# y2w-oc/CMR-Agent

Hardware: AMD Instinct MI355X
Metric: registration iters/sec (KITTI 352x1216 img + 16384 pts, 1 geo forward + 10 agent steps) (higher is better)
Workload: dtype f32; 1 GPU; BASELINE.json configs[1]: KittiConfig, batch 8 per GPU, 16384 pts, 352x1216 image, 10 agent steps, fp32, hash-filled weights; batch_per_gpu=8, parallelism=batch sharding, no data-path collective

## Files before the change

cmr_agent_amd/csrc/agent.hip:

```cpp
#include "cmr_common.h"

namespace {

__global__ __launch_bounds__(256) void project_scatter_kernel(const float* __restrict__ pc4, const float* __restrict__ feat,
                                                              const uint8_t* __restrict__ overlap,
                                                              const float* __restrict__ pose ,
                                                              const float* __restrict__ Kmat ,
                                                              const float* __restrict__ mean4 ,
                                                              float* __restrict__ acc, float* __restrict__ cnt,
                                                              float* __restrict__ state3d, int B, int N, int h, int w) {
  const int lane = threadIdx.x & 63;
  const int64_t p0 = ((int64_t)blockIdx.x * 4 + (threadIdx.x >> 6)) * 4;
  const int64_t total = (int64_t)B * N;
  for (int q = 0; q < 4; ++q) {
    const int64_t p = p0 + q;
    if (p >= total) return;
    const int b = (int)(p / N);
    const f32x4 pt = *reinterpret_cast<const f32x4*>(pc4 + p * 4);
    const float* R = pose + b * 16;
    const float* Kb = Kmat + b * 9;
    const float mx = mean4[b * 4 + 0], my = mean4[b * 4 + 1], mz = mean4[b * 4 + 2];
    const float cx = pt[0] - mx, cy = pt[1] - my, cz = pt[2] - mz;
    const float tx = (R[0] * cx + R[1] * cy + R[2] * cz) + mx + R[3];
    const float ty = (R[4] * cx + R[5] * cy + R[6] * cz) + my + R[7];
// ... 46 lines not shown
__device__ __forceinline__ void obs_mark_reach(uint8_t* __restrict__ map, int r, int b, int yi, int xi, int h, int w) {
  const int tiles_y = (h + 7) >> 3, tiles_x = (w + 15) >> 4;
  const int ya = (yi - r > 0 ? yi - r : 0) >> 3, yb = (yi + r) >> 3 < tiles_y ? (yi + r) >> 3 : tiles_y - 1;
  const int xa = (xi - r > 0 ? xi - r : 0) >> 4, xb = (xi + r) >> 4 < tiles_x ? (xi + r) >> 4 : tiles_x - 1;
  uint8_t* m = map + (int64_t)b * tiles_y * tiles_x;
  m[ya * tiles_x + xa] = 1;
  m[ya * tiles_x + xb] = 1;
  m[yb * tiles_x + xa] = 1;
  m[yb * tiles_x + xb] = 1;
}

__global__ __launch_bounds__(256) void obs_project_kernel(const float* __restrict__ pc4, const uint8_t* __restrict__ overlap,
                                                          const float* __restrict__ pose, const float* __restrict__ Kmat,
                                                          const float* __restrict__ mean4, float* __restrict__ proj, float* __restrict__ cnt,
                                                          int32_t* __restrict__ cell, float* __restrict__ state3d, int B, int N, int h, int w,
                                                          uint8_t* __restrict__ reach1, uint8_t* __restrict__ reach2) {
  const int64_t p = (int64_t)blockIdx.x * 256 + threadIdx.x;
  if (p >= (int64_t)B * N) return;
  const int32_t prev = cell[p];
  if (prev >= 0) {
    f32x4* row = reinterpret_cast<f32x4*>(proj + (int64_t)prev * 64);
    const f32x4 z = {0.f, 0.f, 0.f, 0.f};
#pragma unroll
    for (int i = 0; i < 16; ++i) row[i] = z;
    cnt[prev] = 0.f;
  }
  const int b = (int)(p / N);
  const f32x4 pt = *reinterpret_cast<const f32x4*>(pc4 + p * 4);
  const float* R = pose + b * 16;
  const float* Kb = Kmat + b * 9;
  const float mx = mean4[b * 4 + 0], my = mean4[b * 4 + 1], mz = mean4[b * 4 + 2];
// ... 6 lines not shown
  const float zc = Kb[6] * tx + Kb[7] * ty + Kb[8] * tz;
  u = u / zc;
  v = v / zc;
  const bool inside = (u >= 0.f) && (u <= (float)(w - 1)) && (v >= 0.f) && (v <= (float)(h - 1)) && (zc > 0.f);
  const bool ov = overlap[p] != 0;
  *reinterpret_cast<f32x4*>(state3d + p * 8) = f32x4{pt[0], pt[1], pt[2], ov ? 1.f : 0.f};
  *reinterpret_cast<f32x4*>(state3d + p * 8 + 4) = f32x4{inside ? 1.f : 0.f, 0.f, 0.f, 0.f};
  int32_t c = -1;
  if (ov && inside) {
    const int xi = (int)rintf(u), yi = (int)rintf(v);
    c = (int32_t)((int64_t)b * h * w + (int64_t)yi * w + xi);
    if (reach1) {
      obs_mark_reach(reach1, 1, b, yi, xi, h, w);
      obs_mark_reach(reach2, 2, b, yi, xi, h, w);
    }
  }
  cell[p] = c;
}

__global__ __launch_bounds__(256) void obs_count_kernel(const int32_t* __restrict__ cell, float* __restrict__ cnt, int64_t total) {
  const int64_t p = (int64_t)blockIdx.x * 256 + threadIdx.x;
  if (p >= total) return;
  const int32_t c = cell[p];
  if (c >= 0) atomicAdd(cnt + c, 1.f);
}

__global__ __launch_bounds__(256) void obs_scatter_kernel(const float* __restrict__ feat, const int32_t* __restrict__ cell,
                                                          const float* __restrict__ cnt, float* __restrict__ proj, int64_t total) {
  const int lane = threadIdx.x & 63;
  const int64_t p0 = ((int64_t)blockIdx.x * 4 + (threadIdx.x >> 6)) * 4;
// ... 107 lines not shown
extern "C" int cmr_project_scatter_f32(const float* pc4, const float* feat, const uint8_t* overlap, const float* pose,
                                       const float* Kmat, const float* mean4, float* acc, float* cnt, float* state3d,
                                       int B, int N, int h, int w, int zero_first, hipStream_t stream) {
  CMR_REQUIRE(pc4 && feat && overlap && pose && Kmat && mean4 && acc && cnt && state3d && B > 0 && N > 0 && h > 0 && w > 0);
  const int64_t cells = (int64_t)B * h * w;
  if (zero_first) {
    if (hipMemsetAsync(acc, 0, cells * 64 * sizeof(float), stream) != hipSuccess) return CMR_ELAUNCH;
    if (hipMemsetAsync(cnt, 0, cells * sizeof(float), stream) != hipSuccess) return CMR_ELAUNCH;
  }
  const int64_t total = (int64_t)B * N;
  hipLaunchKernelGGL(project_scatter_kernel, dim3((unsigned)((total + 15) / 16)), dim3(256), 0, stream, pc4, feat, overlap,
                     pose, Kmat, mean4, acc, cnt, state3d, B, N, h, w);
  return cmr_launch_status();
}

extern "C" int cmr_observation_proj_reach_f32(const float* pc4, const float* feat, const uint8_t* overlap, const float* pose, const float* Kmat,
                                              const float* mean4, float* proj, float* cnt, int32_t* cell, float* state3d, int B, int N, int h,
                                              int w, uint8_t* reach1, uint8_t* reach2, hipStream_t stream) {
  CMR_REQUIRE(pc4 && feat && overlap && pose && Kmat && mean4 && proj && cnt && cell && state3d && B > 0 && N > 0 && h > 0 && w > 0);
  CMR_REQUIRE((int64_t)B * h * w < 0x7fffffff && cmr_aligned16(proj) && cmr_aligned16(state3d) && cmr_aligned16(pc4));
  CMR_REQUIRE((reach1 == nullptr) == (reach2 == nullptr));
  const int64_t total = (int64_t)B * N;
  const unsigned per_point = (unsigned)((total + 255) / 256);
  hipLaunchKernelGGL(obs_project_kernel, dim3(per_point), dim3(256), 0, stream, pc4, overlap, pose, Kmat, mean4, proj, cnt, cell, state3d, B, N,
                     h, w, reach1, reach2);
  hipLaunchKernelGGL(obs_count_kernel, dim3(per_point), dim3(256), 0, stream, (const int32_t*)cell, cnt, total);
  hipLaunchKernelGGL(obs_scatter_kernel, dim3((unsigned)((total + 15) / 16)), dim3(256), 0, stream, feat, (const int32_t*)cell,
                     (const float*)cnt, proj, total);
  return cmr_launch_status();
}

extern "C" int cmr_observation_proj_f32(const float* pc4, const float* feat, const uint8_t* overlap, const float* pose, const float* Kmat,
                                        const float* mean4, float* proj, float* cnt, int32_t* cell, float* state3d, int B, int N, int h,
                                        int w, hipStream_t stream) {
  return cmr_observation_proj_reach_f32(pc4, feat, overlap, pose, Kmat, mean4, proj, cnt, cell, state3d, B, N, h, w, nullptr, nullptr, stream);
}

extern "C" int cmr_observation_finalize_f32(const float* img_feat, float* acc, float* cnt, float* state2d,
                                            float* proj, int B, int h, int w, int write_img, int clear, hipStream_t stream) {
  CMR_REQUIRE(img_feat && acc && cnt && (state2d || proj) && B > 0 && h > 0 && w > 0);
  const int64_t cells = (int64_t)B * h * w;
  hipLaunchKernelGGL(observation_finalize_kernel, dim3((unsigned)((cells * 16 + 255) / 256)), dim3(256), 0, stream,
                     img_feat, acc, cnt, state2d, proj, cells, write_img, clear);
  return cmr_launch_status();
// ... 38 lines not shown
```

cmr_agent_amd/csrc/conv_wino.hip:

```cpp
#include "cmr_common.h"


namespace {

struct WinoArgs {
  const float* x; int B, H, W, Cin;
  const float* u;
  const float* bias; const float* res; const float* post;
  float* y; int Cout; float slope; int pool;
  float* stats;
  const float* bn_x; const float* bn_stat; float bn_slope;
};

constexpr int WT_TH = 8, WT_TW = 16;
constexpr int WT_HR = 10, WT_HC = 18;
constexpr int WT_KC = 32;
constexpr int WT_C4 = WT_KC / 4;
constexpr int WT_HALO_F4 = WT_HR * WT_HC * WT_C4;
constexpr int WT_HL = (WT_HALO_F4 + 255) / 256;
constexpr int WT_PITCH = 20;
constexpr int WT_SLOTS = WT_HR * WT_PITCH;
constexpr int WT_HALO_FLOATS = WT_SLOTS * WT_KC;
constexpr int WT_DMA = WT_SLOTS / 8;
constexpr int WT_DMA_PER_WAVE = (WT_DMA + 3) / 4;
// ... 279 lines not shown
}

constexpr int WS_T_OFF = 2 * WT_HALO_FLOATS;
constexpr int WS_T_ROW = 68;
constexpr int WS_SMEM_FLOATS = WS_T_OFF + 8 * 32 * WS_T_ROW;

__device__ __forceinline__ void ws_barrier_lds() { asm volatile("s_waitcnt lgkmcnt(0)\n\ts_barrier" ::: "memory"); }

#ifndef CMR_WS_STATS
#define CMR_WS_STATS 1
#endif
#ifndef CMR_WS_BNBWD
#define CMR_WS_BNBWD 0
#endif
constexpr bool WS_STATS = CMR_WS_STATS != 0, WS_BNBWD = CMR_WS_STATS != 0 && CMR_WS_BNBWD != 0;
struct WsList { const int* order; const int* nlive; const float* y0; };
template <int dbg, bool LIST>
__global__ __launch_bounds__(512, 1) void conv3x3_wino_ws_kernel(const WinoArgs a, const int tiles_x, const int tiles_y, const int ntiles, const WsList l) {
  extern __shared__ __attribute__((aligned(16))) float smem[];
  constexpr int NT = 2;
  constexpr int NMW = 4;
  const int tid = threadIdx.x, lane = tid & 63;
  const int wave = __builtin_amdgcn_readfirstlane(tid >> 6);
  const int nco = a.Cout / 64;
  const int nchunk = a.Cin / WT_KC;
  int nt = ntiles;
  if constexpr (LIST) {
    nt = __builtin_amdgcn_readfirstlane(*l.nlive);
    nt = nt < 0 ? 0 : (nt < ntiles ? nt : ntiles);
  }
  const int nk = (nt - (int)blockIdx.x + (int)gridDim.x - 1) / (int)gridDim.x;
// ... 397 lines not shown
        st_s[e] += cmr_xhalf(st_s[e]);
        st_q[e] += cmr_xor16(st_q[e]);
        st_q[e] += cmr_xhalf(st_q[e]);
      }
      if (lane < 16) {
        float* o = a.stats + ((int64_t)blockIdx.x * 4 + hw) * 128 + 4 * lane;
        *reinterpret_cast<f32x4*>(o) = st_s;
        *reinterpret_cast<f32x4*>(o + 64) = st_q;
      }
    }
  }
  if constexpr (LIST) {
    const int pw = a.pool == 2 ? WT_TW / 2 : WT_TW, pn = a.pool == 2 ? WT_TH * WT_TW / 4 : WT_TH * WT_TW;
    const int Hy = a.pool == 2 ? a.H >> 1 : a.H, Wy = a.pool == 2 ? a.W >> 1 : a.W;
    const int c4 = tid & 15;
    for (int s = nt + (int)blockIdx.x; s < ntiles; s += (int)gridDim.x) {
      int t = l.order[s];
      t = (unsigned)t < (unsigned)ntiles ? t : ntiles - 1;
      const int co0 = (t % nco) * 64; t /= nco;
      const int bx0 = (t % tiles_x) * pw; t /= tiles_x;
      const int by0 = (t % tiles_y) * (pn / pw);
      const int b = t / tiles_y;
      for (int p = tid >> 4; p < pn; p += 32) {
        const int py = by0 + p / pw, px = bx0 + p % pw;
        if (py >= Hy || px >= Wy) continue;
        const int64_t o = (((int64_t)b * Hy + py) * Wy + px) * a.Cout + co0 + 4 * c4;
        f32x4 v;
        if (l.y0) {
          v = *reinterpret_cast<const f32x4*>(l.y0 + o);
        } else {
          const f32x4 bsv = *reinterpret_cast<const f32x4*>(a.bias ? a.bias + co0 + 4 * c4 : wt_zero16);
// ... 134 lines not shown
    const int v = tid >= d ? cnt[tid - d] : 0;
    __syncthreads();
    cnt[tid] += v;
    __syncthreads();
  }
  const int total = cnt[1023];
  int live = cnt[tid] - n, dead = total + (lo - live);
  for (int i = lo; i < hi; ++i) {
    const int slot = reach[i] != 0 ? live++ : dead++;
    reach[i] = 0;
    for (int c = 0; c < nco; ++c) order[slot * nco + c] = i * nco + c;
  }
  if (tid == 0) *(blockIdx.x ? nlive2 : nlive1) = total * nco;
}

}

extern "C" int cmr_wino_tile_lists(uint8_t* reach1, uint8_t* reach2, int B, int H, int W, int Cout1, int Cout2, int* order1, int* nlive1,
                                   int* order2, int* nlive2, hipStream_t stream) {
  CMR_REQUIRE(reach1 && reach2 && order1 && nlive1 && order2 && nlive2 && B > 0 && H > 0 && W > 0);
  CMR_REQUIRE(Cout1 >= 64 && Cout1 % 64 == 0 && Cout2 >= 64 && Cout2 % 64 == 0);
  const int64_t ntile = (int64_t)((W + WT_TW - 1) / WT_TW) * ((H + WT_TH - 1) / WT_TH) * B;
  CMR_REQUIRE(ntile * (Cout1 / 64) < 0x3fffffff && ntile * (Cout2 / 64) < 0x3fffffff);
  hipLaunchKernelGGL(wino_tile_lists_kernel, dim3(2), dim3(1024), 0, stream, reach1, reach2, (int)ntile, Cout1 / 64, Cout2 / 64, order1, nlive1,
                     order2, nlive2);
  return cmr_launch_status();
}

extern "C" int cmr_conv3x3_wino_list_nhwc_f32(const float* x, int B, int H, int W, int Cin, const float* u, const float* bias, const float* res,
                                              float* y, int Cout, float slope, int pool, const int* order, const int* nlive, const float* y0,
                                              int cu_budget, int slices, hipStream_t stream) {
  CMR_REQUIRE(x && u && y && order && nlive && B > 0 && H > 0 && W > 0 && Cin % 32 == 0 && Cin >= 32 && Cout % 64 == 0 && Cout >= 64);
  CMR_REQUIRE(cmr_aligned16(x) && cmr_aligned16(u) && cmr_aligned16(y) && (!bias || cmr_aligned16(bias)) && (!res || cmr_aligned16(res)) &&
              (!y0 || cmr_aligned16(y0)));
  CMR_REQUIRE((pool == 1 || (pool == 2 && !res && y0)) && y0 != y);
  const int tiles_x = (W + WT_TW - 1) / WT_TW, tiles_y = (H + WT_TH - 1) / WT_TH;
  const int64_t ntiles64 = (int64_t)tiles_x * tiles_y * B * (Cout / 64);
  CMR_REQUIRE(2 * ntiles64 < 0x7fffffff);
  if (!(CMR_WINO_WS && Cin >= 64 && ntiles64 >= 200 && slope >= 0.f && slope <= 1.f)) return CMR_EUNSUPPORTED;
  const WinoArgs a{x, B, H, W, Cin, u, bias, res, nullptr, y, Cout, slope, pool};
  return launch_wino_ws_t<0, true>(a, tiles_x, tiles_y, ntiles64, cu_budget, slices, stream, WsList{order, nlive, y0});
}
```

cmr_agent_amd/environment/environment.py:

```python
import torch

from .. import ops
from ..models.CMRAgent import CMRAgent
from ..models.ImageResNet import to_nhwc
from ..models.PointNN import rows_from_bcl


DIRECT_PROJ = True


class _ObsContext:

    def __init__(self, data):
        cl = data.get('_cmr')
        pc = data['pc']
        self.B, _, self.N = pc.shape
        dev = pc.device
        if cl is not None and 'geo' in cl and cl['geo'].pc4.device == dev:
            self.pc4 = cl['geo'].pc4
        else:
            self.pc4 = ops.planar_to_rows(pc.contiguous(), 4)
        self.feat = cl['pc_geo_feat'] if cl is not None and 'pc_geo_feat' in cl else rows_from_bcl(data['pc_geo_feat'])
        ov = data['pc_overlap_pred']
        self.overlap = ov.contiguous().view(torch.uint8).view(-1) if ov.dtype == torch.bool else ov.to(torch.uint8).view(-1)
        self.overlap_src = ov
        self.img = cl['img_geo_feat'] if cl is not None and 'img_geo_feat' in cl else to_nhwc(data['img_geo_feat'])
        _, self.h, self.w, c = self.img.shape
        if c != 64:
            raise ValueError("observation kernels are instantiated for 64-d geometric features")
        self.K = data['K'].to(dev).contiguous()
        cen = data.get('_cmr_centroid')
        self.mean4 = cen[1] if (cen is not None and cen[0] is pc) else _centroid(pc, self.pc4)
        self.acc = self.cnt = None
        self.first = True
        self.proj = self.proj_cnt = self.proj_cell = None
        self.reach, self.obs_serial = None, 0
        self.agent_cache = {}
        self.dirty = False


def _context(data):
    ctx = data.get('_cmr_obs')
    if ctx is None or ctx.overlap_src is not data['pc_overlap_pred'] or ctx.pc4.device != data['pc'].device:
        ctx = _ObsContext(data)
        data['_cmr_obs'] = ctx
    return ctx


def _centroid(pcd, pc4=None):
    B, _, N = pcd.shape
# ... 30 lines not shown
    return poses


@torch.no_grad()
def observation_from_a_pose(data, RT, materialize_state_2d=True):
    ctx = _context(data)
    B, N, h, w = ctx.B, ctx.N, ctx.h, ctx.w
    dev = ctx.pc4.device
    state3d = torch.empty((B * N, 8), dtype=torch.float32, device=dev)
    if not materialize_state_2d and DIRECT_PROJ:
        if ctx.proj is None:
            ctx.proj = torch.zeros((B, h, w, 64), dtype=torch.float32, device=dev)
            ctx.proj_cnt = torch.zeros((B * h * w,), dtype=torch.float32, device=dev)
            ctx.proj_cell = torch.full((B * N,), -1, dtype=torch.int32, device=dev)
        sparse = CMRAgent.sparse_obs()
        if sparse and ctx.reach is None:
            ctx.reach = torch.zeros((2, B, (h + 7) // 8, (w + 15) // 16), dtype=torch.uint8, device=dev)
        ops.observation_proj(ctx.pc4, ctx.feat, ctx.overlap, RT.contiguous(), ctx.K, ctx.mean4, B, N, h, w, ctx.proj, ctx.proj_cnt,
                             ctx.proj_cell, state3d, reach=ctx.reach if sparse else None)
        ctx.obs_serial += 1
        ctx.agent_cache["reach"] = (ctx.reach, ctx.proj, ctx.obs_serial) if sparse else None
        obs2d = torch.empty((B, 128, h, w), dtype=torch.float32, device="meta")
        obs2d._cmr_split = (ctx.img, ctx.proj, ctx.agent_cache)
        return obs2d, state3d.view(B, N, 8)[:, :, :5].permute(0, 2, 1)
    state2d = torch.empty((B, h, w, 128), dtype=torch.float32, device=dev) if materialize_state_2d else None
    proj = torch.empty((B, h, w, 64), dtype=torch.float32, device=dev)
    if ctx.acc is None:
        ctx.acc = torch.zeros((B * h * w, 64), dtype=torch.float32, device=dev)
        ctx.cnt = torch.zeros((B * h * w,), dtype=torch.float32, device=dev)
    zero_first, ctx.dirty = ctx.dirty, True
    ops.project_scatter(ctx.pc4, ctx.feat, ctx.overlap, RT.contiguous(), ctx.K, ctx.mean4, B, N, h, w, ctx.acc, ctx.cnt,
                        state3d, zero_first=zero_first)
    ops.observation_finalize(ctx.img, ctx.acc, ctx.cnt, state2d, proj, B, h, w, True, clear=True)
    ctx.dirty = False
    obs2d = state2d.permute(0, 3, 1, 2) if state2d is not None else torch.empty((B, 128, h, w), dtype=torch.float32, device="meta")
    obs2d._cmr_split = (ctx.img, proj, ctx.agent_cache)
# ... 52 lines not shown
```

cmr_agent_amd/models/CMRAgent.py:

```python
import torch
import torch.nn as nn

from .. import ops
from ..utils.streams import fork_join
from . import _pack
from ._pack import Planned
from .ImageResNet import to_nhwc
from .PointNN import ConvBNReLURes1D

SLOPE = 0.01


def _mlp(sizes):
    layers = []
    for i in range(len(sizes) - 1):
        layers.append(nn.Linear(sizes[i], sizes[i + 1]))
        if i < len(sizes) - 2:
            layers.append(nn.LeakyReLU(inplace=True))
    return nn.Sequential(*layers)


class CMRAgent(Planned):
    def __init__(self, config):
        super().__init__()
# ... 66 lines not shown
                g = ops.colmax_partials(part, B, N // 32)
                b1b = ops.linear(g, ent["w1b"], ent["b1"])
                b2b = ops.linear(g, ent["wscb"], ent["b2"])
            last = i == 2
            r = ops.cbr_block(feat, ent["w1a"], b1b, ent["w2"], b2b, ent["wsca"], 0.2, rows_per_batch=N,
                              want_y=not last, want_colmax="partials")
            if r is None:
                return None
            feat, part = r
        return ops.colmax_partials(part, B, N // 32)

    FUSED_TAIL = True
    TAIL_T = True

    SPARSE_OBS = True

    @classmethod
    def sparse_obs(cls):
        return cls.SPARSE_OBS and ops.WINOGRAD and not ops.CONV_BF16

    def _tile_lists(self, cache, proj, c, u0, u1):
        mark = cache.get("reach")
        if mark is None or not self.sparse_obs() or self.training or mark[1] is not proj or u0 is None or u1 is None:
            return None
        B, h, w, cin = proj.shape
        if h % 2 or w % 2 or not (ops.wino_list_served(B, h, w, cin, c) and ops.wino_list_served(B, h, w, c, c)):
            return None
        if cache.get("lists_of") != mark[2]:
            cache["lists"] = (c, ops.wino_tile_lists(mark[0], B, h, w, c, c))
            cache["lists_of"] = mark[2]
        width, lists = cache["lists"]
        return lists if width == c else None

    def _embed_2d(self, state2d, B, split):
        p = self.plan()
        c = 2 * self.config.embed_dim
        x = state2d
        for stage, ((wa, ba, ua), (wb, bb, ub)) in enumerate(p["convs"]):
            if stage == 0 and split is not None:
                img_src, proj, cache = split
                tag = (id(self), id(p))
                if cache.get("tag") != tag:
                    wi, bi, ui = p["conv0_img"]
                    cache["val"] = ops.conv3x3(img_src, wi, bi, c, 1, 1.0, u=ui)
                    cache["tag"] = tag
                wp, _, up = p["conv0_proj"]
                lists = self._tile_lists(cache, proj, c, up, ub)
                if lists is not None:
                    if cache.get("tag0") != tag:
                        none = torch.zeros((1,), dtype=torch.int32, device=proj.device)
                        cache["x1_0"] = ops.conv3x3_wino_list(proj, up, None, c, SLOPE, lists[0][0], none, None, res=cache["val"])
                        cache["x2_0"] = ops.conv3x3(cache["x1_0"], wb, bb, c, 1, SLOPE, pool=2, u=ub)
                        cache["tag0"] = tag
                    (o1, n1), (o2, n2) = lists
                    x = ops.conv3x3_wino_list(proj, up, None, c, SLOPE, o1, n1, cache["x1_0"], res=cache["val"])
                    x = ops.conv3x3_wino_list(x, ub, bb, c, SLOPE, o2, n2, cache["x2_0"], pool=2)
                    continue
                x = ops.conv3x3(proj, wp, None, c, 1, SLOPE, res=cache["val"], u=up, out_bf16=True)
            else:
                x = ops.conv3x3(x, wa, ba, c, 1, SLOPE, u=ua, out_bf16=True)
            x = ops.conv3x3(x, wb, bb, c, 1, SLOPE, pool=2 if stage < 3 else 1, u=ub, out_bf16=stage < 3)
            if stage == 3:
                kh, kw = self.config.image_H // 8, self.config.image_W // 8
                if (x.shape[1], x.shape[2]) != (kh, kw):
                    raise ValueError("state_2d is %dx%d at the global pool, config says %dx%d" % (x.shape[1], x.shape[2], kh, kw))
        return x

    def _embed_3d_any(self, state3d_rows, B, N):
        e3d = self._embed_3d(state3d_rows, B, N)
        if e3d is None:
            layers = self.state_3d_embed
            feat = layers[0].rows(state3d_rows)
            for i in (1, 2, 3):
# ... 88 lines not shown
```

cmr_agent_amd/ops.py:

```python
import collections
import math
import os

import numpy as np
import torch

from . import _lib

ACT_NONE, ACT_RELU, ACT_LRELU, ACT_GELU, ACT_ELU1 = 0, 1, 2, 3, 4
f32 = torch.float32
GRID_Y_MAX = 65535


def _stream():
    return torch.cuda.current_stream().cuda_stream


def _p(t):
    return None if t is None else t.data_ptr()


def _rows(t, name="tensor"):
    if t.dim() != 2 or t.stride(1) != 1 or t.dtype != f32 or not t.is_cuda:
        raise ValueError("%s must be a 2-D float32 device tensor with unit inner stride, got %s %s %s" % (
# ... 189 lines not shown
def conv3x3_wino_list(x, u, bias, cout, slope, order, nlive, y0, res=None, pool=1):
    B, H, W, cin = x.shape
    hp, wp = (H // 2, W // 2) if pool == 2 else (H, W)
    ntiles = ((W + 15) // 16) * ((H + 7) // 8) * B * (cout // 64)
    if not x.is_contiguous() or x.dtype != f32 or tuple(u.shape) != (16, cout, cin):
        raise ValueError("conv3x3_wino_list: bad operand layout")
    if order.dtype != torch.int32 or nlive.dtype != torch.int32 or order.numel() != ntiles or nlive.numel() != 1 or not order.is_contiguous():
        raise ValueError("conv3x3_wino_list: order must be int32 [%d] and nlive int32 [1]" % ntiles)
    if (y0 is not None and (tuple(y0.shape) != (B, hp, wp, cout) or not y0.is_contiguous() or y0.dtype != f32)) or (
            res is not None and (tuple(res.shape) != (B, H, W, cout) or not res.is_contiguous() or res.dtype != f32)):
        raise ValueError("conv3x3_wino_list: y0 / res of the wrong shape")
    y = torch.empty((B, hp, wp, cout), dtype=f32, device=x.device)
    _lib.call("cmr_conv3x3_wino_list_nhwc_f32", _p(x), B, H, W, cin, _p(u), _p(bias), _p(res), _p(y), cout, float(slope), pool, _p(order),
              _p(nlive), _p(y0), _cu_budget(), _slices(), _stream())
    return y


def wino_tile_lists(reach, B, H, W, cout1, cout2):
    nt = B * ((H + 7) // 8) * ((W + 15) // 16)
    if reach.dtype != torch.uint8 or reach.numel() != 2 * nt or not reach.is_contiguous():
        raise ValueError("wino_tile_lists: reach must be uint8 [2, %d]" % nt)
    n1, n2 = nt * (cout1 // 64), nt * (cout2 // 64)
    buf = torch.empty((n1 + n2 + 8,), dtype=torch.int32, device=reach.device)
    o1, o2, l1, l2 = buf[:n1], buf[n1:n1 + n2], buf[n1 + n2:n1 + n2 + 1], buf[n1 + n2 + 4:n1 + n2 + 5]
    _lib.call("cmr_wino_tile_lists", _p(reach), reach.data_ptr() + nt, B, H, W, cout1, cout2, _p(o1), _p(l1), _p(o2), _p(l2), _stream())
    return (o1, l1), (o2, l2)


def conv3x3_wino_stats(x, u, bias, cout):
    B, H, W, cin = x.shape
# ... 537 lines not shown
def project_scatter(pc4, feat, overlap_u8, pose, K, mean4, B, N, h, w, acc, cnt, state3d, zero_first=True):
    _lib.call("cmr_project_scatter_f32", _p(pc4), _p(feat), _p(overlap_u8), _p(pose), _p(K), _p(mean4), _p(acc), _p(cnt),
              _p(state3d), B, N, h, w, int(zero_first), _stream())


def observation_finalize(img_feat, acc, cnt, state2d, proj, B, h, w, write_img, clear=False):
    _lib.call("cmr_observation_finalize_f32", _p(img_feat), _p(acc), _p(cnt), _p(state2d), _p(proj), B, h, w,
              int(write_img), int(clear), _stream())


def observation_proj(pc4, feat, overlap_u8, pose, K, mean4, B, N, h, w, proj, cnt, cell, state3d, reach=None):
    if cell.dtype != torch.int32 or cell.numel() != B * N or proj.numel() != B * h * w * 64 or cnt.numel() != B * h * w:
        raise ValueError("observation_proj: state buffers of the wrong shape / dtype")
    if reach is not None:
        nt = B * ((h + 7) // 8) * ((w + 15) // 16)
        if reach.dtype != torch.uint8 or reach.numel() != 2 * nt or not reach.is_contiguous():
            raise ValueError("observation_proj: reach must be uint8 [2, %d]" % nt)
        _lib.call("cmr_observation_proj_reach_f32", _p(pc4), _p(feat), _p(overlap_u8), _p(pose), _p(K), _p(mean4), _p(proj), _p(cnt), _p(cell),
                  _p(state3d), B, N, h, w, _p(reach), reach.data_ptr() + nt, _stream())
        return
    _lib.call("cmr_observation_proj_f32", _p(pc4), _p(feat), _p(overlap_u8), _p(pose), _p(K), _p(mean4), _p(proj), _p(cnt), _p(cell), _p(state3d),
              B, N, h, w, _stream())


def pose_step(pose, act_r, act_t, r_steps, t_steps, six_dof):
    _lib.call("cmr_pose_step_f32", _p(pose), _p(act_r), _p(act_t), _p(r_steps), _p(t_steps), pose.shape[0], int(six_dof),
              _stream())


def to_disentangled(pose, mean4):
# ... 1494 lines not shown
```

include/cmr_hip.h:

```cpp
#ifndef CMR_HIP_H
#define CMR_HIP_H
#include <stdint.h>

#ifdef __cplusplus
extern "C" {
#endif

typedef struct ihipStream_t* hipStream_t;

#define CMR_OK 0
#define CMR_EINVAL -1
#define CMR_ELAUNCH -2
#define CMR_EUNSUPPORTED -3

enum { CMR_ACT_NONE = 0, CMR_ACT_RELU = 1, CMR_ACT_LRELU = 2, CMR_ACT_GELU = 3, CMR_ACT_ELU1 = 4 };


int cmr_linear_f32(const float* x1, int64_t ld1, int k1, const float* x2, int64_t ld2, int k2, const int32_t* idx2,
                   int64_t div2, const float* w, int64_t ldw, const float* bias, const float* res, int64_t ldres,
                   int64_t res_mod, float* y, int64_t ldy, int64_t rows, int n_out, int act, float act_param,
                   hipStream_t stream);
int cmr_cbr_block_f32(const float* x1, int64_t ld1, int k1, const float* x2, int64_t ld2, const int32_t* idx2,
                      int64_t div2, int kx, int ch, int co, const float* w1, const float* b1, int64_t b1_stride,
                      const float* w2, const float* b2, int64_t b2_stride, const float* wsc, float* y, int64_t ldy,
// ... 9 lines not shown
int cmr_layernorm64_f32(const float* x, int64_t ldx, const float* gamma, const float* beta, float eps, const float* res,
                        int64_t ldres, float* y, int64_t ldy, int64_t rows, hipStream_t stream);

int cmr_conv3x3_nhwc_f32(const float* x, int B, int H, int W, int Cin, const float* w, const float* bias,
                         const float* res, const float* post, float* y, int Cout, int stride, float slope, int pool,
                         hipStream_t stream);

int cmr_conv3x3_wino_nhwc_f32(const float* x, int B, int H, int W, int Cin, const float* u, const float* bias,
                              const float* res, const float* post, float* y, int Cout, float slope, int pool,
                              int cu_budget, int slices, hipStream_t stream);
int cmr_conv3x3_wino_list_nhwc_f32(const float* x, int B, int H, int W, int Cin, const float* u, const float* bias, const float* res,
                                   float* y, int Cout, float slope, int pool, const int* order, const int* nlive, const float* y0,
                                   int cu_budget, int slices, hipStream_t stream);
int cmr_wino_tile_lists(uint8_t* reach1, uint8_t* reach2, int B, int H, int W, int Cout1, int Cout2, int* order1, int* nlive1,
                        int* order2, int* nlive2, hipStream_t stream);
int64_t cmr_conv3x3_wino_stats_parts(int B, int H, int W, int Cin, int Cout, int cu_budget, int slices);
int cmr_conv3x3_wino_stats_nhwc_f32(const float* x, int B, int H, int W, int Cin, const float* u, const float* bias, float* y, int Cout,
                                    int cu_budget, int slices, float* part, int64_t parts, hipStream_t stream);
int cmr_conv3x3_wino_bnbwd_nhwc_f32(const float* dy, int B, int H, int W, int Cin, const float* u, float* dx, int Cout, const float* bn_x,
                                    const float* bn_stat, float bn_slope, int cu_budget, int slices, float* part, int64_t parts,
                                    hipStream_t stream);
int cmr_conv3x3_s2_nhwc_f32(const float* x, int B, int H, int W, int Cin, const float* wfrag, const float* bias, const float* res,
                            const float* post, float* y, int Cout, float slope, hipStream_t stream);
int cmr_stem_block_f32(const float* x_nchw, const float* w_a, const float* b_a, const float* w3, const float* w1,
                       const float* b_b, float* tmp_nchw, void* y_nhwc, int out_bf16, int B, int H, int W, float slope,
                       hipStream_t stream);

int cmr_avgpool_nhwc_f32(const float* x, float* y, int B, int H, int W, int C, int kh, int kw, hipStream_t stream);

int cmr_upsample_concat_f32(const float* f, const float* proxy, float* out, int B, int H, int W, int C1, int C2,
// ... 246 lines not shown
int cmr_colmean_f32(const float* x, int64_t ldx, float* out, void* ws, int64_t ws_bytes, int B, int N, int C,
                    hipStream_t stream);


int cmr_project_scatter_f32(const float* pc4, const float* feat, const uint8_t* overlap, const float* pose,
                            const float* Kmat, const float* mean4, float* acc, float* cnt, float* state3d, int B, int N,
                            int h, int w, int zero_first, hipStream_t stream);
int cmr_observation_finalize_f32(const float* img_feat, float* acc, float* cnt, float* state2d, float* proj,
                                 int B, int h, int w, int write_img, int clear, hipStream_t stream);
int cmr_observation_proj_f32(const float* pc4, const float* feat, const uint8_t* overlap, const float* pose, const float* Kmat,
                             const float* mean4, float* proj, float* cnt, int32_t* cell, float* state3d, int B, int N, int h, int w,
                             hipStream_t stream);
int cmr_observation_proj_reach_f32(const float* pc4, const float* feat, const uint8_t* overlap, const float* pose, const float* Kmat,
                                   const float* mean4, float* proj, float* cnt, int32_t* cell, float* state3d, int B, int N, int h, int w,
                                   uint8_t* reach1, uint8_t* reach2, hipStream_t stream);
int cmr_pose_step_f32(float* pose, const int64_t* act_r, const int64_t* act_t, const double* r_steps,
                      const double* t_steps, int B, int six_dof, hipStream_t stream);
int cmr_to_disentangled_f32(float* pose, const float* mean4, int B, hipStream_t stream);
int cmr_argmax_rows_f32(const float* x, int64_t* out, int outer, int inner, int n, int64_t stride_outer,
                        int64_t stride_inner, hipStream_t stream);
int cmr_softmax2_f32(const float* logits, int64_t ld, float* prob, uint8_t* pred_lo, uint8_t* pred_hi, float thr_lo,
                     float thr_hi, int64_t rows, hipStream_t stream);
int cmr_l2norm64_f32(const float* x, int64_t ldx, float* y, int64_t ldy, int64_t rows, hipStream_t stream);


int64_t cmr_bn_workspace_bytes(int64_t rows, int C);
int cmr_bn_stats_f32(const float* x, int64_t ldx, int64_t rows, int C, float eps, float momentum, const float* gamma,
                     const float* beta, float* running_mean, float* running_var, float* stat, void* ws, int64_t ws_bytes,
                     hipStream_t stream);
int cmr_bn_bwd_from_sums_f32(const float* dz, int64_t lddz, float slope, const float* x, int64_t ldx, const float* stat, const float* part,
// ... 221 lines not shown
```

Baseline: 475.9 registration iters/s.

## Reuse previous-step conv outputs in place and restore only tiles that changed

Sparse observation convs now write into persistent per-step output buffers and track which tiles were live in the previous step. A new list kernel partitions tiles into live, restore (live last step but not now, copied back from the baseline output) and dead, so each step no longer rewrites every untouched tile from y0. Optional stage-1 sparsity with half-resolution reach maps is added but disabled by default. This adds state across agent steps and more bookkeeping, with a risk of stale outputs if the tracking is wrong.

Result: faster. 492.4 registration iters/s, median of 6 (+3.5%).

```diff
diff --git a/cmr_agent_amd/csrc/agent.hip b/cmr_agent_amd/csrc/agent.hip
--- a/cmr_agent_amd/csrc/agent.hip
+++ b/cmr_agent_amd/csrc/agent.hip
@@ -84,7 +84,8 @@
                                                           const float* __restrict__ pose, const float* __restrict__ Kmat,
                                                           const float* __restrict__ mean4, float* __restrict__ proj, float* __restrict__ cnt,
                                                           int32_t* __restrict__ cell, float* __restrict__ state3d, int B, int N, int h, int w,
-                                                          uint8_t* __restrict__ reach1, uint8_t* __restrict__ reach2) {
+                                                          uint8_t* __restrict__ reach1, uint8_t* __restrict__ reach2,
+                                                          uint8_t* __restrict__ reach3, uint8_t* __restrict__ reach4) {
   const int64_t p = (int64_t)blockIdx.x * 256 + threadIdx.x;
   if (p >= (int64_t)B * N) return;
   const int32_t prev = cell[p];
@@ -121,6 +122,10 @@
       obs_mark_reach(reach1, 1, b, yi, xi, h, w);
       obs_mark_reach(reach2, 2, b, yi, xi, h, w);
     }
+    if (reach3) {
+      obs_mark_reach(reach3, 2, b, yi >> 1, xi >> 1, h >> 1, w >> 1);
+      obs_mark_reach(reach4, 3, b, yi >> 1, xi >> 1, h >> 1, w >> 1);
+    }
   }
   cell[p] = c;
 }
@@ -258,20 +263,28 @@
   return cmr_launch_status();
 }
 
+extern "C" int cmr_observation_proj_reach4_f32(const float* pc4, const float* feat, const uint8_t* overlap, const float* pose, const float* Kmat,
+                                               const float* mean4, float* proj, float* cnt, int32_t* cell, float* state3d, int B, int N, int h,
+                                               int w, uint8_t* reach1, uint8_t* reach2, uint8_t* reach3, uint8_t* reach4, hipStream_t stream) {
+  CMR_REQUIRE(pc4 && feat && overlap && pose && Kmat && mean4 && proj && cnt && cell && state3d && B > 0 && N > 0 && h > 0 && w > 0);
+  CMR_REQUIRE((int64_t)B * h * w < 0x7fffffff && cmr_aligned16(proj) && cmr_aligned16(state3d) && cmr_aligned16(pc4));
+  CMR_REQUIRE((reach1 == nullptr) == (reach2 == nullptr) && (reach3 == nullptr) == (reach4 == nullptr));
+  CMR_REQUIRE(!reach3 || (reach1 && h % 2 == 0 && w % 2 == 0));
+  const int64_t total = (int64_t)B * N;
+  const unsigned per_point = (unsigned)((total + 255) / 256);
+  hipLaunchKernelGGL(obs_project_kernel, dim3(per_point), dim3(256), 0, stream, pc4, overlap, pose, Kmat, mean4, proj, cnt, cell, state3d, B, N,
+                     h, w, reach1, reach2, reach3, reach4);
+  hipLaunchKernelGGL(obs_count_kernel, dim3(per_point), dim3(256), 0, stream, (const int32_t*)cell, cnt, total);
+  hipLaunchKernelGGL(obs_scatter_kernel, dim3((unsigned)((total + 15) / 16)), dim3(256), 0, stream, feat, (const int32_t*)cell,
+                     (const float*)cnt, proj, total);
+  return cmr_launch_status();
+}
+
 extern "C" int cmr_observation_proj_reach_f32(const float* pc4, const float* feat, const uint8_t* overlap, const float* pose, const float* Kmat,
                                               const float* mean4, float* proj, float* cnt, int32_t* cell, float* state3d, int B, int N, int h,
                                               int w, uint8_t* reach1, uint8_t* reach2, hipStream_t stream) {
-  CMR_REQUIRE(pc4 && feat && overlap && pose && Kmat && mean4 && proj && cnt && cell && state3d && B > 0 && N > 0 && h > 0 && w > 0);
-  CMR_REQUIRE((int64_t)B * h * w < 0x7fffffff && cmr_aligned16(proj) && cmr_aligned16(state3d) && cmr_aligned16(pc4));
-  CMR_REQUIRE((reach1 == nullptr) == (reach2 == nullptr));
-  const int64_t total = (int64_t)B * N;
-  const unsigned per_point = (unsigned)((total + 255) / 256);
-  hipLaunchKernelGGL(obs_project_kernel, dim3(per_point), dim3(256), 0, stream, pc4, overlap, pose, Kmat, mean4, proj, cnt, cell, state3d, B, N,
-                     h, w, reach1, reach2);
-  hipLaunchKernelGGL(obs_count_kernel, dim3(per_point), dim3(256), 0, stream, (const int32_t*)cell, cnt, total);
-  hipLaunchKernelGGL(obs_scatter_kernel, dim3((unsigned)((total + 15) / 16)), dim3(256), 0, stream, feat, (const int32_t*)cell,
-                     (const float*)cnt, proj, total);
-  return cmr_launch_status();
+  return cmr_observation_proj_reach4_f32(pc4, feat, overlap, pose, Kmat, mean4, proj, cnt, cell, state3d, B, N, h, w, reach1, reach2, nullptr,
+                                         nullptr, stream);
 }
 
 extern "C" int cmr_observation_proj_f32(const float* pc4, const float* feat, const uint8_t* overlap, const float* pose, const float* Kmat,
diff --git a/cmr_agent_amd/csrc/conv_wino.hip b/cmr_agent_amd/csrc/conv_wino.hip
--- a/cmr_agent_amd/csrc/conv_wino.hip
+++ b/cmr_agent_amd/csrc/conv_wino.hip
@@ -317,7 +317,7 @@
 #define CMR_WS_BNBWD 0
 #endif
 constexpr bool WS_STATS = CMR_WS_STATS != 0, WS_BNBWD = CMR_WS_STATS != 0 && CMR_WS_BNBWD != 0;
-struct WsList { const int* order; const int* nlive; const float* y0; };
+struct WsList { const int* order; const int* nlive; const float* y0; const int* nrestore; };
 template <int dbg, bool LIST>
 __global__ __launch_bounds__(512, 1) void conv3x3_wino_ws_kernel(const WinoArgs a, const int tiles_x, const int tiles_y, const int ntiles, const WsList l) {
   extern __shared__ __attribute__((aligned(16))) float smem[];
@@ -745,7 +745,12 @@
     const int pw = a.pool == 2 ? WT_TW / 2 : WT_TW, pn = a.pool == 2 ? WT_TH * WT_TW / 4 : WT_TH * WT_TW;
     const int Hy = a.pool == 2 ? a.H >> 1 : a.H, Wy = a.pool == 2 ? a.W >> 1 : a.W;
     const int c4 = tid & 15;
-    for (int s = nt + (int)blockIdx.x; s < ntiles; s += (int)gridDim.x) {
+    int end = ntiles;
+    if (l.nrestore) {
+      const int nr = __builtin_amdgcn_readfirstlane(*l.nrestore);
+      end = nr < 0 ? nt : (nr < ntiles - nt ? nt + nr : ntiles);
+    }
+    for (int s = nt + (int)blockIdx.x; s < end; s += (int)gridDim.x) {
       int t = l.order[s];
       t = (unsigned)t < (unsigned)ntiles ? t : ntiles - 1;
       const int co0 = (t % nco) * 64; t /= nco;
@@ -910,6 +915,66 @@
   if (tid == 0) *(blockIdx.x ? nlive2 : nlive1) = total * nco;
 }
 
+struct WsListJob { uint8_t* reach; uint8_t* prev; int* order; int* counts; int ntile; };
+struct WsListJobs { WsListJob j[4]; };
+__global__ __launch_bounds__(1024) void wino_tile_lists_obs_kernel(const WsListJobs jobs, int nco) {
+  __shared__ int cl[1024], cr[1024];
+  const WsListJob j = jobs.j[blockIdx.x];
+  const int tid = threadIdx.x, ntile = j.ntile;
+  const int per = (ntile + 1023) / 1024;
+  const int lo = tid * per < ntile ? tid * per : ntile, hi = lo + per < ntile ? lo + per : ntile;
+  int nl = 0, nr = 0;
+  for (int i = lo; i < hi; ++i) {
+    const bool lv = j.reach[i] != 0;
+    nl += lv;
+    nr += !lv && (!j.prev || j.prev[i] != 0);
+  }
+  cl[tid] = nl;
+  cr[tid] = nr;
+  __syncthreads();
+  for (int d = 1; d < 1024; d <<= 1) {
+    const int vl = tid >= d ? cl[tid - d] : 0, vr = tid >= d ? cr[tid - d] : 0;
+    __syncthreads();
+    cl[tid] += vl;
+    cr[tid] += vr;
+    __syncthreads();
+  }
+  const int tl = cl[1023], tr = cr[1023];
+  int live = cl[tid] - nl, rest = cr[tid] - nr;
+  int dead = tl + tr + (lo - live - rest);
+  rest += tl;
+  for (int i = lo; i < hi; ++i) {
+    const bool lv = j.reach[i] != 0, rs = !lv && (!j.prev || j.prev[i] != 0);
+    const int slot = lv ? live++ : (rs ? rest++ : dead++);
+    if (j.prev) j.prev[i] = lv;
+    j.reach[i] = 0;
+    for (int c = 0; c < nco; ++c) j.order[slot * nco + c] = i * nco + c;
+  }
+  if (tid == 0) {
+    j.counts[0] = tl * nco;
+    j.counts[1] = tr * nco;
+  }
+}
+
+}
+
+extern "C" int cmr_wino_tile_lists_obs(uint8_t* reach, uint8_t* prev, int nmaps, int B, int H, int W, int Cout, int* order, int* counts,
+                                       hipStream_t stream) {
+  CMR_REQUIRE(reach && order && counts && B > 0 && H > 0 && W > 0 && Cout >= 64 && Cout % 64 == 0);
+  CMR_REQUIRE(nmaps == 2 || (nmaps == 4 && H % 2 == 0 && W % 2 == 0));
+  const int nco = Cout / 64;
+  const int64_t nt0 = (int64_t)((W + WT_TW - 1) / WT_TW) * ((H + WT_TH - 1) / WT_TH) * B;
+  const int64_t nt1 = (int64_t)((W / 2 + WT_TW - 1) / WT_TW) * ((H / 2 + WT_TH - 1) / WT_TH) * B;
+  CMR_REQUIRE(nt0 * nco < 0x3fffffff);
+  WsListJobs jobs{};
+  int64_t at = 0;
+  for (int m = 0; m < nmaps; ++m) {
+    const int64_t nt = m < 2 ? nt0 : nt1;
+    jobs.j[m] = WsListJob{reach + at, prev ? prev + at : nullptr, order + at * nco, counts + 2 * m, (int)nt};
+    at += nt;
+  }
+  hipLaunchKernelGGL(wino_tile_lists_obs_kernel, dim3((unsigned)nmaps), dim3(1024), 0, stream, jobs, nco);
+  return cmr_launch_status();
 }
 
 extern "C" int cmr_wino_tile_lists(uint8_t* reach1, uint8_t* reach2, int B, int H, int W, int Cout1, int Cout2, int* order1, int* nlive1,
@@ -923,9 +988,9 @@
   return cmr_launch_status();
 }
 
-extern "C" int cmr_conv3x3_wino_list_nhwc_f32(const float* x, int B, int H, int W, int Cin, const float* u, const float* bias, const float* res,
-                                              float* y, int Cout, float slope, int pool, const int* order, const int* nlive, const float* y0,
-                                              int cu_budget, int slices, hipStream_t stream) {
+static int wino_list_call(const float* x, int B, int H, int W, int Cin, const float* u, const float* bias, const float* res, float* y, int Cout,
+                          float slope, int pool, const int* order, const int* nlive, const int* nrestore, const float* y0, int cu_budget,
+                          int slices, hipStream_t stream) {
   CMR_REQUIRE(x && u && y && order && nlive && B > 0 && H > 0 && W > 0 && Cin % 32 == 0 && Cin >= 32 && Cout % 64 == 0 && Cout >= 64);
   CMR_REQUIRE(cmr_aligned16(x) && cmr_aligned16(u) && cmr_aligned16(y) && (!bias || cmr_aligned16(bias)) && (!res || cmr_aligned16(res)) &&
               (!y0 || cmr_aligned16(y0)));
@@ -935,5 +1000,18 @@
   CMR_REQUIRE(2 * ntiles64 < 0x7fffffff);
   if (!(CMR_WINO_WS && Cin >= 64 && ntiles64 >= 200 && slope >= 0.f && slope <= 1.f)) return CMR_EUNSUPPORTED;
   const WinoArgs a{x, B, H, W, Cin, u, bias, res, nullptr, y, Cout, slope, pool};
-  return launch_wino_ws_t<0, true>(a, tiles_x, tiles_y, ntiles64, cu_budget, slices, stream, WsList{order, nlive, y0});
-}
+  return launch_wino_ws_t<0, true>(a, tiles_x, tiles_y, ntiles64, cu_budget, slices, stream, WsList{order, nlive, y0, nrestore});
+}
+
+extern "C" int cmr_conv3x3_wino_list_nhwc_f32(const float* x, int B, int H, int W, int Cin, const float* u, const float* bias, const float* res,
+                                              float* y, int Cout, float slope, int pool, const int* order, const int* nlive, const float* y0,
+                                              int cu_budget, int slices, hipStream_t stream) {
+  return wino_list_call(x, B, H, W, Cin, u, bias, res, y, Cout, slope, pool, order, nlive, nullptr, y0, cu_budget, slices, stream);
+}
+
+extern "C" int cmr_conv3x3_wino_list_restore_nhwc_f32(const float* x, int B, int H, int W, int Cin, const float* u, const float* bias,
+                                                      const float* res, float* y, int Cout, float slope, int pool, const int* order,
+                                                      const int* counts, const float* y0, int cu_budget, int slices, hipStream_t stream) {
+  CMR_REQUIRE(counts && y0);
+  return wino_list_call(x, B, H, W, Cin, u, bias, res, y, Cout, slope, pool, order, counts, counts + 1, y0, cu_budget, slices, stream);
+}
diff --git a/cmr_agent_amd/environment/environment.py b/cmr_agent_amd/environment/environment.py
--- a/cmr_agent_amd/environment/environment.py
+++ b/cmr_agent_amd/environment/environment.py
@@ -34,6 +34,7 @@
         self.acc = self.cnt = None
         self.first = True
         self.proj = self.proj_cnt = self.proj_cell = None
+        self.reach_maps = 0
         self.reach, self.obs_serial = None, 0
         self.agent_cache = {}
         self.dirty = False
@@ -94,12 +95,14 @@
             ctx.proj_cnt = torch.zeros((B * h * w,), dtype=torch.float32, device=dev)
             ctx.proj_cell = torch.full((B * N,), -1, dtype=torch.int32, device=dev)
         sparse = CMRAgent.sparse_obs()
-        if sparse and ctx.reach is None:
-            ctx.reach = torch.zeros((2, B, (h + 7) // 8, (w + 15) // 16), dtype=torch.uint8, device=dev)
+        nmaps = CMRAgent.sparse_obs_maps(B, h, w) if sparse else 0
+        if sparse and (ctx.reach is None or ctx.reach_maps != nmaps):
+            ctx.reach = torch.zeros((2 * sum(ops.obs_tile_counts(B, h, w, nmaps)),), dtype=torch.uint8, device=dev)
+            ctx.reach_maps = nmaps
         ops.observation_proj(ctx.pc4, ctx.feat, ctx.overlap, RT.contiguous(), ctx.K, ctx.mean4, B, N, h, w, ctx.proj, ctx.proj_cnt,
                              ctx.proj_cell, state3d, reach=ctx.reach if sparse else None)
         ctx.obs_serial += 1
-        ctx.agent_cache["reach"] = (ctx.reach, ctx.proj, ctx.obs_serial) if sparse else None
+        ctx.agent_cache["reach"] = (ctx.reach, ctx.proj, ctx.obs_serial, nmaps) if sparse else None
         obs2d = torch.empty((B, 128, h, w), dtype=torch.float32, device="meta")
         obs2d._cmr_split = (ctx.img, ctx.proj, ctx.agent_cache)
         return obs2d, state3d.view(B, N, 8)[:, :, :5].permute(0, 2, 1)
diff --git a/cmr_agent_amd/models/CMRAgent.py b/cmr_agent_amd/models/CMRAgent.py
--- a/cmr_agent_amd/models/CMRAgent.py
+++ b/cmr_agent_amd/models/CMRAgent.py
@@ -104,12 +104,18 @@
     TAIL_T = True
 
     SPARSE_OBS = True
+    SPARSE_OBS_STAGE1 = False
+    SPARSE_OBS_INPLACE = True
 
     @classmethod
     def sparse_obs(cls):
         return cls.SPARSE_OBS and ops.WINOGRAD and not ops.CONV_BF16
 
-    def _tile_lists(self, cache, proj, c, u0, u1):
+    @classmethod
+    def sparse_obs_maps(cls, B, h, w):
+        return 4 if cls.SPARSE_OBS_STAGE1 and h % 2 == 0 and w % 2 == 0 else 2
+
+    def _tile_lists(self, cache, proj, c, u0, u1, key):
         mark = cache.get("reach")
         if mark is None or not self.sparse_obs() or self.training or mark[1] is not proj or u0 is None or u1 is None:
             return None
@@ -117,15 +123,28 @@
         if h % 2 or w % 2 or not (ops.wino_list_served(B, h, w, cin, c) and ops.wino_list_served(B, h, w, c, c)):
             return None
         if cache.get("lists_of") != mark[2]:
-            cache["lists"] = (c, ops.wino_tile_lists(mark[0], B, h, w, c, c))
+            if cache.get("tag0") != key:
+                cache["prev"] = torch.ones_like(mark[0]) if self.SPARSE_OBS_INPLACE else None
+                cache["restore_all_of"] = mark[2]
+            lists = ops.wino_tile_lists_obs(mark[0], cache["prev"], mark[3], B, h, w, c)
+            if len(lists) == 4 and not ops.wino_list_served(B, h // 2, w // 2, c, c):
+                lists = lists[:2]
+            cache["lists"] = (c, lists)
             cache["lists_of"] = mark[2]
         width, lists = cache["lists"]
         return lists if width == c else None
+
+    def _list_conv(self, cache, key, x, u, bias, c, lst, y0, res=None, pool=1):
+        order, nlive, counts = lst
+        if cache.get("prev") is None:
+            return ops.conv3x3_wino_list(x, u, bias, c, SLOPE, order, nlive, y0, res=res, pool=pool)
+        return ops.conv3x3_wino_list_restore(x, u, bias, c, SLOPE, order, counts, y0, cache[key], res=res, pool=pool)
 
     def _embed_2d(self, state2d, B, split):
         p = self.plan()
         c = 2 * self.config.embed_dim
         x = state2d
+        sparse1 = None
         for stage, ((wa, ba, ua), (wb, bb, ub)) in enumerate(p["convs"]):
             if stage == 0 and split is not None:
                 img_src, proj, cache = split
@@ -135,18 +154,35 @@
                     cache["val"] = ops.conv3x3(img_src, wi, bi, c, 1, 1.0, u=ui)
                     cache["tag"] = tag
                 wp, _, up = p["conv0_proj"]
-                lists = self._tile_lists(cache, proj, c, up, ub)
+                key0 = (tag, self.SPARSE_OBS_INPLACE, cache["reach"][3] if cache.get("reach") else 0)
+                lists = self._tile_lists(cache, proj, c, up, ub, key0)
                 if lists is not None:
-                    if cache.get("tag0") != tag:
+                    if cache.get("tag0") != key0:
                         none = torch.zeros((1,), dtype=torch.int32, device=proj.device)
                         cache["x1_0"] = ops.conv3x3_wino_list(proj, up, None, c, SLOPE, lists[0][0], none, None, res=cache["val"])
                         cache["x2_0"] = ops.conv3x3(cache["x1_0"], wb, bb, c, 1, SLOPE, pool=2, u=ub)
-                        cache["tag0"] = tag
-                    (o1, n1), (o2, n2) = lists
-                    x = ops.conv3x3_wino_list(proj, up, None, c, SLOPE, o1, n1, cache["x1_0"], res=cache["val"])
-                    x = ops.conv3x3_wino_list(x, ub, bb, c, SLOPE, o2, n2, cache["x2_0"], pool=2)
+                        if len(lists) == 4:
+                            (w3, b3, u3), (w4, b4, u4) = p["convs"][1]
+                            cache["x3_0"] = ops.conv3x3(cache["x2_0"], w3, b3, c, 1, SLOPE, u=u3)
+                            cache["x4_0"] = ops.conv3x3(cache["x3_0"], w4, b4, c, 1, SLOPE, pool=2, u=u4)
+                        if cache.get("prev") is not None:
+                            for k in ("y1", "y2", "y3", "y4")[:len(lists)]:
+                                cache[k] = torch.empty_like(cache["x" + k[1] + "_0"])
+                                if cache.get("restore_all_of") != cache["lists_of"]:
+                                    cache[k].copy_(cache["x" + k[1] + "_0"])
+                        cache["tag0"] = key0
+                    x = self._list_conv(cache, "y1", proj, up, None, c, lists[0], cache["x1_0"], res=cache["val"])
+                    x = self._list_conv(cache, "y2", x, ub, bb, c, lists[1], cache["x2_0"], pool=2)
+                    sparse1 = (cache, lists[2:]) if len(lists) == 4 else None
                     continue
                 x = ops.conv3x3(proj, wp, None, c, 1, SLOPE, res=cache["val"], u=up, out_bf16=True)
+            elif stage == 1 and sparse1 is not None:
+                cache, (la, lb) = sparse1
+                if ua is None or ub is None:
+                    raise ValueError("sparse observation: stage 1 has no Winograd weights")
+                x = self._list_conv(cache, "y3", x, ua, ba, c, la, cache["x3_0"])
+                x = self._list_conv(cache, "y4", x, ub, bb, c, lb, cache["x4_0"], pool=2)
+                continue
             else:
                 x = ops.conv3x3(x, wa, ba, c, 1, SLOPE, u=ua, out_bf16=True)
             x = ops.conv3x3(x, wb, bb, c, 1, SLOPE, pool=2 if stage < 3 else 1, u=ub, out_bf16=stage < 3)
diff --git a/cmr_agent_amd/ops.py b/cmr_agent_amd/ops.py
--- a/cmr_agent_amd/ops.py
+++ b/cmr_agent_amd/ops.py
@@ -227,6 +227,50 @@
     _lib.call("cmr_conv3x3_wino_list_nhwc_f32", _p(x), B, H, W, cin, _p(u), _p(bias), _p(res), _p(y), cout, float(slope), pool, _p(order),
               _p(nlive), _p(y0), _cu_budget(), _slices(), _stream())
     return y
+
+
+def conv3x3_wino_list_restore(x, u, bias, cout, slope, order, counts, y0, y, res=None, pool=1):
+    B, H, W, cin = x.shape
+    hp, wp = (H // 2, W // 2) if pool == 2 else (H, W)
+    ntiles = ((W + 15) // 16) * ((H + 7) // 8) * B * (cout // 64)
+    if not x.is_contiguous() or x.dtype != f32 or tuple(u.shape) != (16, cout, cin):
+        raise ValueError("conv3x3_wino_list_restore: bad operand layout")
+    if order.dtype != torch.int32 or counts.dtype != torch.int32 or order.numel() != ntiles or counts.numel() != 2 or not (
+            order.is_contiguous() and counts.is_contiguous()):
+        raise ValueError("conv3x3_wino_list_restore: order must be int32 [%d] and counts int32 [2]" % ntiles)
+    for t in (y0, y):
+        if tuple(t.shape) != (B, hp, wp, cout) or not t.is_contiguous() or t.dtype != f32:
+            raise ValueError("conv3x3_wino_list_restore: y0 / y of the wrong shape")
+    if res is not None and (tuple(res.shape) != (B, H, W, cout) or not res.is_contiguous() or res.dtype != f32):
+        raise ValueError("conv3x3_wino_list_restore: res of the wrong shape")
+    _lib.call("cmr_conv3x3_wino_list_restore_nhwc_f32", _p(x), B, H, W, cin, _p(u), _p(bias), _p(res), _p(y), cout, float(slope), pool,
+              _p(order), _p(counts), _p(y0), _cu_budget(), _slices(), _stream())
+    return y
+
+
+def obs_tile_counts(B, H, W, nmaps):
+    nt0 = B * ((H + 7) // 8) * ((W + 15) // 16)
+    nt1 = B * ((H // 2 + 7) // 8) * ((W // 2 + 15) // 16) if nmaps == 4 else 0
+    return nt0, nt1
+
+
+def wino_tile_lists_obs(reach, prev, nmaps, B, H, W, cout):
+    if nmaps not in (2, 4) or (nmaps == 4 and (H % 2 or W % 2)):
+        raise ValueError("wino_tile_lists_obs: 2 maps, or 4 on an even-sized map")
+    nt0, nt1 = obs_tile_counts(B, H, W, nmaps)
+    for t in (reach, prev):
+        if t is not None and (t.dtype != torch.uint8 or t.numel() != 2 * (nt0 + nt1) or not t.is_contiguous()):
+            raise ValueError("wino_tile_lists_obs: reach / prev must be uint8 [%d]" % (2 * (nt0 + nt1)))
+    nco = cout // 64
+    buf = torch.empty((2 * (nt0 + nt1) * nco + 2 * nmaps,), dtype=torch.int32, device=reach.device)
+    order, counts = buf[:2 * (nt0 + nt1) * nco], buf[2 * (nt0 + nt1) * nco:]
+    _lib.call("cmr_wino_tile_lists_obs", _p(reach), _p(prev), nmaps, B, H, W, cout, _p(order), _p(counts), _stream())
+    out, at = [], 0
+    for m in range(nmaps):
+        n = (nt0 if m < 2 else nt1) * nco
+        out.append((order[at:at + n], counts[2 * m:2 * m + 1], counts[2 * m:2 * m + 2]))
+        at += n
+    return out
 
 
 def wino_tile_lists(reach, B, H, W, cout1, cout2):
@@ -794,6 +838,12 @@
         raise ValueError("observation_proj: state buffers of the wrong shape / dtype")
     if reach is not None:
         nt = B * ((h + 7) // 8) * ((w + 15) // 16)
+        nt1 = obs_tile_counts(B, h, w, 4)[1]
+        if reach.dtype == torch.uint8 and reach.numel() == 2 * (nt + nt1) and reach.is_contiguous() and h % 2 == 0 and w % 2 == 0:
+            a = reach.data_ptr()
+            _lib.call("cmr_observation_proj_reach4_f32", _p(pc4), _p(feat), _p(overlap_u8), _p(pose), _p(K), _p(mean4), _p(proj), _p(cnt),
+                      _p(cell), _p(state3d), B, N, h, w, a, a + nt, a + 2 * nt, a + 2 * nt + nt1, _stream())
+            return
         if reach.dtype != torch.uint8 or reach.numel() != 2 * nt or not reach.is_contiguous():
             raise ValueError("observation_proj: reach must be uint8 [2, %d]" % nt)
         _lib.call("cmr_observation_proj_reach_f32", _p(pc4), _p(feat), _p(overlap_u8), _p(pose), _p(K), _p(mean4), _p(proj), _p(cnt), _p(cell),
diff --git a/include/cmr_hip.h b/include/cmr_hip.h
--- a/include/cmr_hip.h
+++ b/include/cmr_hip.h
@@ -47,6 +47,11 @@
                                    int cu_budget, int slices, hipStream_t stream);
 int cmr_wino_tile_lists(uint8_t* reach1, uint8_t* reach2, int B, int H, int W, int Cout1, int Cout2, int* order1, int* nlive1,
                         int* order2, int* nlive2, hipStream_t stream);
+int cmr_wino_tile_lists_obs(uint8_t* reach, uint8_t* prev, int nmaps, int B, int H, int W, int Cout, int* order, int* counts,
+                            hipStream_t stream);
+int cmr_conv3x3_wino_list_restore_nhwc_f32(const float* x, int B, int H, int W, int Cin, const float* u, const float* bias,
+                                           const float* res, float* y, int Cout, float slope, int pool, const int* order,
+                                           const int* counts, const float* y0, int cu_budget, int slices, hipStream_t stream);
 int64_t cmr_conv3x3_wino_stats_parts(int B, int H, int W, int Cin, int Cout, int cu_budget, int slices);
 int cmr_conv3x3_wino_stats_nhwc_f32(const float* x, int B, int H, int W, int Cin, const float* u, const float* bias, float* y, int Cout,
                                     int cu_budget, int slices, float* part, int64_t parts, hipStream_t stream);
@@ -323,6 +328,9 @@
 int cmr_observation_proj_reach_f32(const float* pc4, const float* feat, const uint8_t* overlap, const float* pose, const float* Kmat,
                                    const float* mean4, float* proj, float* cnt, int32_t* cell, float* state3d, int B, int N, int h, int w,
                                    uint8_t* reach1, uint8_t* reach2, hipStream_t stream);
+int cmr_observation_proj_reach4_f32(const float* pc4, const float* feat, const uint8_t* overlap, const float* pose, const float* Kmat,
+                                    const float* mean4, float* proj, float* cnt, int32_t* cell, float* state3d, int B, int N, int h, int w,
+                                    uint8_t* reach1, uint8_t* reach2, uint8_t* reach3, uint8_t* reach4, hipStream_t stream);
 int cmr_pose_step_f32(float* pose, const int64_t* act_r, const int64_t* act_t, const double* r_steps,
                       const double* t_steps, int B, int six_dof, hipStream_t stream);
 int cmr_to_disentangled_f32(float* pose, const float* mean4, int B, hipStream_t stream);
```
